# chao1224/pytorch_distributed_nn

Hardware: AMD Instinct MI355X
Metric: samples/sec (whole node) ResNet-50 DDP (higher is better)
Workload: dtype bf16; 1 GPU; model=resnet50 (ImageNet layout, 224x224, 1000 classes), global_batch=256, per_gpu_batch=256, image_size=224, parallelism=dp1, optimizer=fused SGD momentum=0.9 wd=5e-5, hipgraph=False, opt_overlap=False

## Files before the change

### csrc/kernels/conv3x3.hip

```cpp
#include "conv_direct.h"

namespace {
using namespace pg;

typedef __attribute__((ext_vector_type(8))) int c3v8i;
typedef __attribute__((ext_vector_type(4))) int c3v4i;
constexpr int C3_AMAX_PARTS = 1024;
#ifndef C3_PRE_J
#define C3_PRE_J 3
#endif
#ifndef C3_F8_PRE_J
#define C3_F8_PRE_J 2
#endif

template <int FMT>
__device__ __forceinline__ uint4 c3_to_fp8(const float* v) {
    constexpr float MX = FMT ? 57344.f : 448.f;
    int w[4];
#pragma unroll
    for (int d = 0; d < 4; ++d) {
        const float c0 = fminf(fmaxf(v[4 * d], -MX), MX), c1 = fminf(fmaxf(v[4 * d + 1], -MX), MX);
        const float c2 = fminf(fmaxf(v[4 * d + 2], -MX), MX), c3 = fminf(fmaxf(v[4 * d + 3], -MX), MX);
        int x = 0;
        if constexpr (FMT) {
            x = __builtin_amdgcn_cvt_pk_bf8_f32(c0, c1, x, false);
            x = __builtin_amdgcn_cvt_pk_bf8_f32(c2, c3, x, true);
        } else {
            x = __builtin_amdgcn_cvt_pk_fp8_f32(c0, c1, x, false);
            x = __builtin_amdgcn_cvt_pk_fp8_f32(c2, c3, x, true);
        }
        w[d] = x;
    }
    return make_uint4((uint32_t)w[0], (uint32_t)w[1], (uint32_t)w[2], (uint32_t)w[3]);
}

template <int NB, int EPI, bool PRE, int F8 = 0, bool FP = false>
__global__ void __launch_bounds__(256, 2) conv3x3_kernel(C3Args a) {
    constexpr int FN = NB / 16;
    constexpr int BCH = NB * 8 / 256;
    extern __shared__ __attribute__((aligned(16))) char smem[];
    bf16_t* const halo = reinterpret_cast<bf16_t*>(smem);
    bf16_t* const bbuf = halo + (a.halo_max + 1) * 64;

    const int tid = threadIdx.x, lane = tid & 63, wave = tid >> 6;
    const int t = xcd_remap(blockIdx.x, a.tiles * a.ntiles);
    const int tile = t / a.ntiles, nt = t - tile * a.ntiles;
    const int p0 = tile * C3_BM, n0 = nt * NB;
    const int plast = min(a.P, p0 + C3_BM) - 1;
    const int gr0 = (int)fdiv((uint32_t)p0, a.dW), gr1 = (int)fdiv((uint32_t)plast, a.dW);
    const int nrows = gr1 - gr0 + 3;
    const int hpx = nrows * a.W;
    const long gp0 = (long)(gr0 - 1) * a.W;

    int hb[4], py[4], px[4];
    bool pv[4];
#pragma unroll
    for (int f = 0; f < 4; ++f) {
        const int p = p0 + wave * 64 + f * 16 + (lane & 15);
        pv[f] = p < a.P;
        const int pp = pv[f] ? p : plast;
        const int gr = (int)fdiv((uint32_t)pp, a.dW);
        px[f] = pp - gr * a.W;
        py[f] = gr - (int)fdiv((uint32_t)gr, a.dH) * a.H;
        hb[f] = (gr - gr0 + 1) * a.W + px[f];
    }

    [[maybe_unused]] uint32_t tmask[4];
    if constexpr (F8 != 0) {
#pragma unroll
        for (int f = 0; f < 4; ++f) {
            uint32_t m = 0;
#pragma unroll
            for (int tap = 0; tap < 9; ++tap) {
                const int dr = tap / 3 - 1, ds = tap % 3 - 1;
                if (pv[f] && (unsigned)(py[f] + dr) < (unsigned)a.H && (unsigned)(px[f] + ds) < (unsigned)a.W) m |= 1u << tap;
            }
            tmask[f] = m;
        }
    }
    const int zpx = a.halo_max;
    if (tid < 8) *reinterpret_cast<u16x8_t*>(halo + zpx * 64 + tid * 8) = c3_zero8();

    f32x4_t acc[4][FN];
#pragma unroll
    for (int i = 0; i < 4; ++i)
#pragma unroll
        for (int j = 0; j < FN; ++j) acc[i][j] = f32x4_t{0.f, 0.f, 0.f, 0.f};

    const int nchunks = F8 ? a.C >> 7 : a.C >> 6;
    const long wrow = 9L * a.C;
    u16x8_t rb[BCH];
    [[maybe_unused]] const uint8_t* wb8 =
        reinterpret_cast<const uint8_t*>(a.w) + (long)(n0 + (tid >> 3)) * wrow + (tid & 7) * 16;
    auto load_b = [&](int c0, int tap) {
#pragma unroll
        for (int i = 0; i < BCH; ++i) {
            const int li = tid + 256 * i, row = li >> 3, q = li & 7;
            if constexpr (F8 != 0)
                rb[i] = *reinterpret_cast<const u16x8_t*>(wb8 + (long)(32 * i) * wrow + (long)tap * a.C + c0);
            else
                rb[i] = *reinterpret_cast<const u16x8_t*>(a.w + (long)(n0 + row) * wrow + (long)tap * a.C + c0 + q * 8);
        }
    };
    auto store_b = [&](int buf) {
        bf16_t* B = bbuf + buf * NB * 64;
#pragma unroll
        for (int i = 0; i < BCH; ++i) {
            const int li = tid + 256 * i, row = li >> 3, q = li & 7;
            *reinterpret_cast<u16x8_t*>(B + kimg_off(row, q)) = rb[i];
        }
    };

    [[maybe_unused]] float qs = 0.f, amx = 0.f;
    if constexpr (F8 != 0) qs = a.f8_scale[0];

    for (int ck = 0; ck < nchunks; ++ck) {
        const int c0 = F8 ? ck << 7 : ck << 6;
        if (ck) __syncthreads();
        const int nch = hpx * 8;
        if constexpr (F8 != 0) {
            constexpr int J = PRE ? C3_F8_PRE_J : 4;
            [[maybe_unused]] float* coef = reinterpret_cast<float*>(bbuf + NB * 64);
            if constexpr (PRE) {
                pre_coef_lds<128>(a, c0, coef, tid);
                __syncthreads();
            } else if constexpr (FP) {
                fpro_coef_lds<128>(a, c0, coef, tid);
                __syncthreads();
            }
            for (int i0 = 0; i0 < nch; i0 += 256 * J) {
                u16x8_t v[J][2], tv[PRE ? J : 1][2];
                bool okj[J];
                int gpj[J];
#pragma unroll
                for (int j = 0; j < J; ++j) {
                    const int i = i0 + j * 256 + tid;
                    const long gp = gp0 + (i >> 3);
                    okj[j] = i < nch && gp >= 0 && gp < a.P;
                    const long gc = gp < 0 ? 0 : (gp >= a.P ? a.P - 1 : gp);
                    gpj[j] = (int)gc;
                    const bf16_t* src = a.x + gc * a.C + c0 + (i & 7) * 16;
                    v[j][0] = *reinterpret_cast<const u16x8_t*>(src);
                    v[j][1] = *reinterpret_cast<const u16x8_t*>(src + 8);
                    if constexpr (PRE) {
                        const bf16_t* ts = a.pre_t + gc * a.C + c0 + (i & 7) * 16;
                        tv[j][0] = *reinterpret_cast<const u16x8_t*>(ts);
                        tv[j][1] = *reinterpret_cast<const u16x8_t*>(ts + 8);
                    }
                }
#pragma unroll
                for (int j = 0; j < J; ++j) {
                    if constexpr (PRE) {
#pragma unroll
                        for (int h = 0; h < 2; ++h) {
                            v[j][h] = pre_apply_lds<128>(coef, (tid & 7) * 16 + 8 * h, v[j][h], tv[j][h]);
                            if (a.pre_out && nt == 0 && okj[j] && gpj[j] >= p0 && gpj[j] <= plast)
                                *reinterpret_cast<u16x8_t*>(a.pre_out + (long)gpj[j] * a.C + c0 + (tid & 7) * 16 + 8 * h) =
                                    v[j][h];
                        }
                    }
                    if constexpr (FP) {
                        v[j][0] = fpro_apply_lds<128>(coef, (tid & 7) * 16, v[j][0]);
                        v[j][1] = fpro_apply_lds<128>(coef, (tid & 7) * 16 + 8, v[j][1]);
                    }
                    float f[16];
                    unpack8(v[j][0], f);
                    unpack8(v[j][1], f + 8);
                    float m = 0.f;
#pragma unroll
                    for (int e = 0; e < 16; ++e) {
                        m = fmaxf(m, fabsf(f[e]));
                        f[e] *= qs;
                    }
                    if (okj[j]) amx = fmaxf(amx, m);
                    const uint4 q8 = c3_to_fp8<F8 - 1>(f);
                    const int i = i0 + j * 256 + tid;
                    const int off = i < nch ? halo_off(i >> 3, i & 7) : zpx * 64 + (i & 7) * 8;
                    *reinterpret_cast<u16x8_t*>(halo + off) = mask16(__builtin_bit_cast(u16x8_t, q8), okj[j]);
                }
            }
            load_b(c0, 0);
            store_b(0);
            __syncthreads();
            const int g = lane >> 4;
#pragma unroll 1
            for (int tap = 0; tap < 9; ++tap) {
                const int dr = tap / 3 - 1, ds = tap - (tap / 3) * 3 - 1;
                load_b(c0, tap < 8 ? tap + 1 : 8);
                const bf16_t* B = bbuf + (tap & 1) * NB * 64;
                c3v8i bq[FN];
#pragma unroll
                for (int f = 0; f < FN; ++f) {
                    const int row = f * 16 + (lane & 15);
                    const c3v4i lo = *reinterpret_cast<const c3v4i*>(B + kimg_off(row, 2 * g));
                    const c3v4i hi = *reinterpret_cast<const c3v4i*>(B + kimg_off(row, 2 * g + 1));
                    bq[f] = c3v8i{lo[0], lo[1], lo[2], lo[3], hi[0], hi[1], hi[2], hi[3]};
                }
#pragma unroll
                for (int fm = 0; fm < 4; ++fm) {
                    const bool v = (tmask[fm] >> tap) & 1;
                    const int hp = v ? hb[fm] + dr * a.W + ds : zpx;
                    const c3v4i lo = *reinterpret_cast<const c3v4i*>(halo + halo_off(hp, 2 * g));
                    const c3v4i hi = *reinterpret_cast<const c3v4i*>(halo + halo_off(hp, 2 * g + 1));
                    const c3v8i af = c3v8i{lo[0], lo[1], lo[2], lo[3], hi[0], hi[1], hi[2], hi[3]};
#pragma unroll
                    for (int fn = 0; fn < FN; ++fn)
                        acc[fm][fn] = __builtin_amdgcn_mfma_scale_f32_16x16x128_f8f6f4(
                            bq[fn], af, acc[fm][fn], 0, F8 - 1, 0, 0x7f7f7f7f, 0, 0x7f7f7f7f);
                }
                store_b((tap + 1) & 1);
                __syncthreads();
            }
            continue;
        }
        constexpr int J = PRE ? (NB == 128 ? C3_PRE_J : 4) : 8;
        [[maybe_unused]] float* coef = reinterpret_cast<float*>(bbuf + NB * 64);
        if constexpr (PRE) {
            pre_coef_lds<64>(a, c0, coef, tid);
            __syncthreads();
        } else if constexpr (FP) {
            fpro_coef_lds<64>(a, c0, coef, tid);
            __syncthreads();
        }
        for (int i0 = 0; i0 < nch; i0 += 256 * J) {
            u16x8_t v[J], tv[PRE ? J : 1];
            bool okj[J];
            int gpj[J];
#pragma unroll
            for (int j = 0; j < J; ++j) {
                const int i = i0 + j * 256 + tid;
                const long gp = gp0 + (i >> 3);
                okj[j] = i < nch && gp >= 0 && gp < a.P;
                const long gc = gp < 0 ? 0 : (gp >= a.P ? a.P - 1 : gp);
                gpj[j] = (int)gc;
                v[j] = *reinterpret_cast<const u16x8_t*>(a.x + gc * a.C + c0 + (i & 7) * 8);
                if constexpr (PRE) tv[j] = *reinterpret_cast<const u16x8_t*>(a.pre_t + gc * a.C + c0 + (i & 7) * 8);
            }
#pragma unroll
            for (int j = 0; j < J; ++j) {
                if constexpr (PRE) {
                    v[j] = pre_apply_lds<64>(coef, (tid & 7) * 8, v[j], tv[j]);
                    if (a.pre_out && nt == 0 && okj[j] && gpj[j] >= p0 && gpj[j] <= plast)
                        *reinterpret_cast<u16x8_t*>(a.pre_out + (long)gpj[j] * a.C + c0 + (tid & 7) * 8) = v[j];
                }
                if constexpr (FP) v[j] = fpro_apply_lds<64>(coef, (tid & 7) * 8, v[j]);
                v[j] = mask16(v[j], okj[j]);
            }
#pragma unroll
            for (int j = 0; j < J; ++j) {
                const int i = i0 + j * 256 + tid;
                const int off = i < nch ? halo_off(i >> 3, i & 7) : zpx * 64 + (i & 7) * 8;
                *reinterpret_cast<u16x8_t*>(halo + off) = v[j];
            }
        }
        load_b(c0, 0);
        store_b(0);
        __syncthreads();
#pragma unroll 1
        for (int tap = 0; tap < 9; ++tap) {
            const int dr = tap / 3 - 1, ds = tap - (tap / 3) * 3 - 1;
            if (tap < 8) load_b(c0, tap + 1);
            int hp[4];
#pragma unroll
            for (int f = 0; f < 4; ++f) {
                const bool v = pv[f] && (unsigned)(py[f] + dr) < (unsigned)a.H && (unsigned)(px[f] + ds) < (unsigned)a.W;
                hp[f] = v ? hb[f] + dr * a.W + ds : zpx;
            }
            const bf16_t* B = bbuf + (tap & 1) * NB * 64;
#pragma unroll 1
            for (int ks = 0; ks < 2; ++ks) {
                bf16x8_t af[4], bfr[FN];
                const int q = ks * 4 + (lane >> 4);
#pragma unroll
                for (int f = 0; f < 4; ++f)
                    af[f] = __builtin_bit_cast(bf16x8_t, *reinterpret_cast<const u16x8_t*>(halo + halo_off(hp[f], q)));
#pragma unroll
                for (int f = 0; f < FN; ++f) bfr[f] = frag_kmajor(B, f * 16 + (lane & 15), ks, lane);
#pragma unroll
                for (int fm = 0; fm < 4; ++fm)
#pragma unroll
                    for (int fn = 0; fn < FN; ++fn)
                        acc[fm][fn] = __builtin_amdgcn_mfma_f32_16x16x32_bf16(bfr[fn], af[fm], acc[fm][fn], 0, 0, 0);
            }
            if (tap < 8) {
                store_b((tap + 1) & 1);
                __syncthreads();
            }
        }
    }

    if constexpr (F8 != 0) {
        amx = wave_max(amx);
        if (lane == 0)
            atomicMax(reinterpret_cast<unsigned int*>(a.f8_amax + (blockIdx.x & (C3_AMAX_PARTS - 1))), __float_as_uint(amx));
        const float gs = a.f8_inv[0] * a.f8_winv[0];
#pragma unroll
        for (int i = 0; i < 4; ++i)
#pragma unroll
            for (int j = 0; j < FN; ++j)
#pragma unroll
                for (int e = 0; e < 4; ++e) acc[i][j][e] *= gs;
    }
    c3_epilogue<NB, EPI>(a, acc, tile, p0, n0, wave, lane, pv);
}

constexpr int C3R_HREG = 16;

template <int EPI>
__global__ void __launch_bounds__(256, 1) conv3x3_w64_kernel(C3Args a) {
    constexpr int NB = 64, FN = 4;
    extern __shared__ __attribute__((aligned(16))) char smem[];
    bf16_t* const halo = reinterpret_cast<bf16_t*>(smem);
    bf16_t* const wres = halo + (a.halo_max + 1) * 64;
    const int tid = threadIdx.x, lane = tid & 63, wave = tid >> 6;
    const int zpx = a.halo_max;

    for (int i = tid; i < 9 * 64 * 8; i += 256) {
        const int tap = i / 512, row = (i >> 3) & 63, q = i & 7;
        *reinterpret_cast<u16x8_t*>(wres + tap * 4096 + kimg_off(row, q)) =
            *reinterpret_cast<const u16x8_t*>(a.w + (long)row * 576 + tap * 64 + q * 8);
    }
    if (tid < 8) *reinterpret_cast<u16x8_t*>(halo + zpx * 64 + tid * 8) = c3_zero8();

    u16x8_t hreg[C3R_HREG];
    auto tile_geom = [&](int tile, int& gr0, int& nch, long& gp0) {
        const int p0 = tile * C3_BM;
        const int plast = min(a.P, p0 + C3_BM) - 1;
        gr0 = (int)fdiv((uint32_t)p0, a.dW);
        const int gr1 = (int)fdiv((uint32_t)plast, a.dW);
        nch = (gr1 - gr0 + 3) * a.W * 8;
        gp0 = (long)(gr0 - 1) * a.W;
    };
    auto fetch = [&](int tile) {
        int gr0, nch;
        long gp0;
        tile_geom(tile, gr0, nch, gp0);
#pragma unroll
        for (int j = 0; j < C3R_HREG; ++j) {
            const int i = j * 256 + tid;
            const long gp = gp0 + (i >> 3);
            const bool ok = i < nch && gp >= 0 && gp < a.P;
            const long gc = gp < 0 ? 0 : (gp >= a.P ? a.P - 1 : gp);
            const u16x8_t ld = *reinterpret_cast<const u16x8_t*>(a.x + gc * 64 + (i & 7) * 8);
            hreg[j] = mask16(ld, ok);
        }
    };
    auto put = [&](int tile) {
        int gr0, nch;
        long gp0;
        tile_geom(tile, gr0, nch, gp0);
#pragma unroll
        for (int j = 0; j < C3R_HREG; ++j) {
            const int i = j * 256 + tid;
            const int off = i < nch ? halo_off(i >> 3, i & 7) : zpx * 64 + (i & 7) * 8;
            *reinterpret_cast<u16x8_t*>(halo + off) = hreg[j];
        }
    };

    int tile = blockIdx.x;
    if (tile < a.tiles) fetch(tile);
    for (; tile < a.tiles; tile += gridDim.x) {
        __syncthreads();
        put(tile);
        __syncthreads();
        const int next = tile + gridDim.x;
        if (next < a.tiles) fetch(next);

        int gr0, nch;
        long gp0;
        tile_geom(tile, gr0, nch, gp0);
        const int p0 = tile * C3_BM;
        const int plast = min(a.P, p0 + C3_BM) - 1;
        int hb[4], py[4], px[4];
        bool pv[4];
#pragma unroll
        for (int f = 0; f < 4; ++f) {
            const int p = p0 + wave * 64 + f * 16 + (lane & 15);
            pv[f] = p < a.P;
            const int pp = pv[f] ? p : plast;
            const int gr = (int)fdiv((uint32_t)pp, a.dW);
            px[f] = pp - gr * a.W;
            py[f] = gr - (int)fdiv((uint32_t)gr, a.dH) * a.H;
            hb[f] = (gr - gr0 + 1) * a.W + px[f];
        }
        f32x4_t acc[4][FN];
#pragma unroll
        for (int i = 0; i < 4; ++i)
#pragma unroll
            for (int j = 0; j < FN; ++j) acc[i][j] = f32x4_t{0.f, 0.f, 0.f, 0.f};
#pragma unroll
        for (int tap = 0; tap < 9; ++tap) {
            const int dr = tap / 3 - 1, ds = tap % 3 - 1;
            int hp[4];
#pragma unroll
            for (int f = 0; f < 4; ++f) {
                const bool v = pv[f] && (unsigned)(py[f] + dr) < (unsigned)a.H && (unsigned)(px[f] + ds) < (unsigned)a.W;
                hp[f] = v ? hb[f] + dr * a.W + ds : zpx;
            }
            const bf16_t* B = wres + tap * 4096;
#pragma unroll
            for (int ks = 0; ks < 2; ++ks) {
                bf16x8_t af[4], bfr[FN];
                const int q = ks * 4 + (lane >> 4);
#pragma unroll
                for (int f = 0; f < 4; ++f)
                    af[f] = __builtin_bit_cast(bf16x8_t, *reinterpret_cast<const u16x8_t*>(halo + halo_off(hp[f], q)));
#pragma unroll
                for (int f = 0; f < FN; ++f) bfr[f] = frag_kmajor(B, f * 16 + (lane & 15), ks, lane);
#pragma unroll
                for (int fm = 0; fm < 4; ++fm)
#pragma unroll
                    for (int fn = 0; fn < FN; ++fn)
                        acc[fm][fn] = __builtin_amdgcn_mfma_f32_16x16x32_bf16(bfr[fn], af[fm], acc[fm][fn], 0, 0, 0);
            }
        }
        c3_epilogue<NB, EPI>(a, acc, tile, p0, 0, wave, lane, pv);
    }
}

template <int KC, int NB, int EPI, bool PRE, bool FP = false>
__global__ void __launch_bounds__(256, 2) conv1x1_areg_kernel(C3Args a) {
    constexpr int FN = NB / 16, NKS = 2 * KC, K = 64 * KC;
    constexpr int BPT = NB * KC * 8 / 256;
    static_assert(BPT >= 1 && NB * KC * 8 % 256 == 0, "weight step must cover the block");
    extern __shared__ __attribute__((aligned(16))) char smem[];
    bf16_t* const bbuf = reinterpret_cast<bf16_t*>(smem);
    const int tid = threadIdx.x, lane = tid & 63, wave = tid >> 6;
    const int groups = a.ntiles;
    const int t = xcd_remap(blockIdx.x, a.tiles * groups);
    const int tile = t / groups, grp = t - tile * groups;
    const int steps = (a.N / NB) / groups;
    const int c00 = grp * steps;
    const int p0 = tile * C3_BM;

    u16x8_t rb[BPT];
    auto load_b = [&](int s) {
        const int n0 = (c00 + s) * NB;
#pragma unroll
        for (int i = 0; i < BPT; ++i) {
            const int li = tid + 256 * i, row = li / (KC * 8), rem = li - row * (KC * 8);
            rb[i] = *reinterpret_cast<const u16x8_t*>(a.w + (long)(n0 + row) * K + rem * 8);
        }
    };
    auto store_b = [&](int buf) {
        bf16_t* B = bbuf + buf * (KC * NB * 64);
#pragma unroll
        for (int i = 0; i < BPT; ++i) {
            const int li = tid + 256 * i, row = li / (KC * 8), rem = li - row * (KC * 8);
            *reinterpret_cast<u16x8_t*>(B + (rem >> 3) * (NB * 64) + kimg_off(row, rem & 7)) = rb[i];
        }
    };
    load_b(0);

    bool pv[4];
    long prow[4];
#pragma unroll
    for (int fm = 0; fm < 4; ++fm) {
        const int p = p0 + wave * 64 + fm * 16 + (lane & 15);
        pv[fm] = p < a.P;
        prow[fm] = (long)(pv[fm] ? p : a.P - 1) * K;
    }
    bf16x8_t af[NKS][4];
    if constexpr (!PRE) {
        [[maybe_unused]] float* coef = reinterpret_cast<float*>(bbuf + 2 * KC * NB * 64);
        if constexpr (FP) {
            for (int c = tid; c < K; c += 256) {
                coef[c] = a.pro_sc[c];
                coef[K + c] = a.pro_sh[c];
            }
            __syncthreads();
        }
#pragma unroll
        for (int ks = 0; ks < NKS; ++ks)
#pragma unroll
            for (int fm = 0; fm < 4; ++fm) {
                u16x8_t v = *reinterpret_cast<const u16x8_t*>(a.x + prow[fm] + ks * 32 + (lane >> 4) * 8);
                if constexpr (FP) v = fpro_apply_lds<K>(coef, ks * 32 + (lane >> 4) * 8, v);
                af[ks][fm] = __builtin_bit_cast(bf16x8_t, v);
            }
    } else {
        float* coef = reinterpret_cast<float*>(bbuf + 2 * KC * NB * 64);
        {
            const float invL = (float)(1.0 / (double)a.P);
            for (int c = tid; c < K; c += 256) {
                const float is = a.pre_invstd[c], kk = (a.pre_gamma ? a.pre_gamma[c] : 1.f) * is;
                const float dg = a.pre_dgamma[c] * invL, db = a.pre_dbeta[c] * invL;
                coef[c] = kk;
                coef[K + c] = -kk * is * dg;
                coef[2 * K + c] = kk * (a.pre_mean[c] * is * dg - db);
            }
        }
        __syncthreads();
        constexpr int GB = KC == 4 ? 2 : (KC == 2 ? 4 : 2);
#pragma unroll
        for (int g0 = 0; g0 < NKS; g0 += GB) {
            u16x8_t v[GB][4], tv[GB][4];
#pragma unroll
            for (int kk = 0; kk < GB; ++kk)
#pragma unroll
                for (int fm = 0; fm < 4; ++fm) {
                    const long off = prow[fm] + (g0 + kk) * 32 + (lane >> 4) * 8;
                    v[kk][fm] = *reinterpret_cast<const u16x8_t*>(a.x + off);
                    tv[kk][fm] = *reinterpret_cast<const u16x8_t*>(a.pre_t + off);
                }
#pragma unroll
            for (int kk = 0; kk < GB; ++kk) {
                const int k = (g0 + kk) * 32 + (lane >> 4) * 8;
                PreCoef pc;
#pragma unroll
                for (int j = 0; j < 8; ++j) {
                    pc.k[j] = coef[k + j];
                    pc.A[j] = coef[K + k + j];
                    pc.B[j] = coef[2 * K + k + j];
                }
#pragma unroll
                for (int fm = 0; fm < 4; ++fm) {
                    const u16x8_t d = pre_apply(pc, v[kk][fm], tv[kk][fm]);
                    if (a.pre_out && grp == 0 && pv[fm]) *reinterpret_cast<u16x8_t*>(a.pre_out + prow[fm] + k) = d;
                    af[g0 + kk][fm] = __builtin_bit_cast(bf16x8_t, d);
                }
            }
        }
    }
    store_b(0);
    __syncthreads();

    for (int s = 0; s < steps; ++s) {
        const bool more = s + 1 < steps;
        if (more) load_b(s + 1);
        const bf16_t* B = bbuf + (s & 1) * (KC * NB * 64);
        f32x4_t acc[4][FN];
#pragma unroll
        for (int i = 0; i < 4; ++i)
#pragma unroll
            for (int j = 0; j < FN; ++j) acc[i][j] = f32x4_t{0.f, 0.f, 0.f, 0.f};
        bf16x8_t bcur[FN], bnxt[FN];
#pragma unroll
        for (int f = 0; f < FN; ++f) bcur[f] = frag_kmajor(B, f * 16 + (lane & 15), 0, lane);
#pragma unroll
        for (int ks = 0; ks < NKS; ++ks) {
            if (ks + 1 < NKS) {
#pragma unroll
                for (int f = 0; f < FN; ++f)
                    bnxt[f] = frag_kmajor(B + ((ks + 1) >> 1) * (NB * 64), f * 16 + (lane & 15), (ks + 1) & 1, lane);
            }
#pragma unroll
            for (int fm = 0; fm < 4; ++fm)
#pragma unroll
                for (int fn = 0; fn < FN; ++fn)
                    acc[fm][fn] = __builtin_amdgcn_mfma_f32_16x16x32_bf16(bcur[fn], af[ks][fm], acc[fm][fn], 0, 0, 0);
            __builtin_amdgcn_sched_barrier(0);
#pragma unroll
            for (int f = 0; f < FN; ++f) bcur[f] = bnxt[f];
        }
        if (more) store_b((s + 1) & 1);
        c3_epilogue<NB, EPI>(a, acc, tile, p0, (c00 + s) * NB, wave, lane, pv);
        if (more) __syncthreads();
    }
}

int c3r_smem(int W);

__global__ void __launch_bounds__(256) conv3x3_flip_kernel(const bf16_t* __restrict__ w, bf16_t* __restrict__ wt,
                                                           int K, int C) {
    const long n = 9L * K * C;
    for (long i = (long)blockIdx.x * 256 + threadIdx.x; i < n; i += (long)gridDim.x * 256) {
        const int c = (int)(i % C);
        const long r1 = i / C;
        const int tap = (int)(r1 % 9);
        const int k = (int)(r1 / 9);
        wt[((long)c * 9 + (8 - tap)) * K + k] = w[i];
    }
}

int c3_halo_max(int W) {
    const int rows = (C3_BM - 1 + W - 1) / W + 1 + 2;
    return rows * W;
}

__global__ void __launch_bounds__(256) conv3x3_flip8_kernel(const uint8_t* __restrict__ w, uint8_t* __restrict__ wt,
                                                            int K, int C) {
    const long n = 9L * K * C;
    for (long i = (long)blockIdx.x * 256 + threadIdx.x; i < n; i += (long)gridDim.x * 256) {
        const int k = (int)(i % K);
        const long r0 = i / K;
        const int tap = (int)(r0 % 9), c = (int)(r0 / 9);
        wt[i] = w[((long)k * 9 + (8 - tap)) * C + c];
    }
}

template <int NB>
int c3_smem(int W) { return (c3_halo_max(W) + 1) * 128 + 2 * NB * 128; }

int c3r_smem(int W) { return (c3_halo_max(W) + 1) * 128 + 9 * 64 * 128; }

template <int EPI>
int c3r_launch(const C3Args& a, hipStream_t st) {
    static int attr_done = 0;
    const int sm = c3r_smem(a.W);
    if (sm > attr_done) {
        (void)hipFuncSetAttribute((const void*)conv3x3_w64_kernel<EPI>, hipFuncAttributeMaxDynamicSharedMemorySize, sm);
        attr_done = sm;
    }
    const int grid = a.tiles < grid_cus() ? a.tiles : grid_cus();
    hipLaunchKernelGGL((conv3x3_w64_kernel<EPI>), dim3(grid), dim3(256), sm, st, a);
    PDNN_LAUNCH_RET;
}

template <int NB, int EPI, bool PRE, int F8 = 0, bool FP = false>
int c3_launch(const C3Args& a, hipStream_t st) {
    static int attr_done = 0;
    const int sm = c3_smem<NB>(a.W);
    if (sm > attr_done) {
        (void)hipFuncSetAttribute((const void*)conv3x3_kernel<NB, EPI, PRE, F8, FP>,
                                  hipFuncAttributeMaxDynamicSharedMemorySize, sm);
        attr_done = sm;
    }
    hipLaunchKernelGGL((conv3x3_kernel<NB, EPI, PRE, F8, FP>), dim3(a.tiles * a.ntiles), dim3(256), sm, st, a);
    PDNN_LAUNCH_RET;
}

template <int NB, bool PRE>
int c3_dispatch(const C3Args& a, int epi, hipStream_t st) {
    switch (epi) {
        case C3_BNB: return c3_launch<NB, C3_BNB, PRE>(a, st);
        case C3_STATS: return c3_launch<NB, C3_STATS, PRE>(a, st);
        case C3_RES: return c3_launch<NB, C3_RES, PRE>(a, st);
        default: return c3_launch<NB, C3_PLAIN, PRE>(a, st);
    }
}

}



template <int KC, int NB, int EPI, bool PRE, bool FP = false>
int areg_launch(const C3Args& a, hipStream_t st) {
    constexpr int sm = 2 * KC * NB * 128 + (PRE ? 3 * 64 * KC * 4 : (FP ? 2 * 64 * KC * 4 : 0));
    hipLaunchKernelGGL((conv1x1_areg_kernel<KC, NB, EPI, PRE, FP>), dim3(a.tiles * a.ntiles), dim3(256), sm, st, a);
    PDNN_LAUNCH_RET;
}

template <int KC, int NB, bool PRE>
int areg_dispatch(const C3Args& a, int epi, hipStream_t st) {
    if constexpr (!PRE) {
        if (a.pro_sc) {
            if (epi == C3_STATS) return areg_launch<KC, NB, C3_STATS, false, true>(a, st);
            if (epi == C3_PLAIN) return areg_launch<KC, NB, C3_PLAIN, false, true>(a, st);
            return (int)hipErrorInvalidValue;
        }
    }
    switch (epi) {
        case C3_BNB: return areg_launch<KC, NB, C3_BNB, PRE>(a, st);
        case C3_STATS: return areg_launch<KC, NB, C3_STATS, PRE>(a, st);
        case C3_RES: return areg_launch<KC, NB, C3_RES, PRE>(a, st);
        default: return areg_launch<KC, NB, C3_PLAIN, PRE>(a, st);
    }
}

template <bool PRE>
int areg_run(C3Args& a, int K, int epi, hipStream_t st) {
    const int nb = K == 256 ? 32 : 64;
    const int chunks = a.N / nb;
    int g = 1;
    while (g < chunks && (long)a.tiles * g < 512 && chunks % (2 * g) == 0) g *= 2;
    a.ntiles = g;
    if (K == 64) return areg_dispatch<1, 64, PRE>(a, epi, st);
    if (K == 128) return areg_dispatch<2, 64, PRE>(a, epi, st);
    return areg_dispatch<4, 32, PRE>(a, epi, st);
}

static bool set_pre(C3Args& a, const bf16_t* t, const float* mean, const float* invstd, const float* gamma,
             const float* dgamma, const float* dbeta, bf16_t* out) {
    a.pre_t = t; a.pre_mean = mean; a.pre_invstd = invstd; a.pre_gamma = gamma;
    a.pre_dgamma = dgamma; a.pre_dbeta = dbeta; a.pre_out = out;
    if (!t) return !out;
    return mean && invstd && dgamma && dbeta;
}
static int c3_force() { return pg::tune().conv3x3_force; }

static FastDiv make_fdiv_c3(uint32_t d) {
    FastDiv f;
    f.d = d ? d : 1;
    uint32_t l = 0;
    while ((1ull << l) < f.d) ++l;
    f.s = l;
    f.m = (uint32_t)((((1ull << l) - f.d) << 32) / f.d + 1);
    return f;
}

PDNN_API int pdnn_conv3x3_supported(int Nimg, int H, int W, int C, int N) {
    if (C % 64 || N % 64 || C < 64 || N < 64 || W < 1 || H < 1) return 0;
    if (W < 12 && !c3_force()) return 0;
    if ((long)Nimg * H * W >= (1L << 31) / 2) return 0;
    const int nb = N % 128 == 0 ? 128 : 64;
    const int sm = nb == 128 ? c3_smem<128>(W) : c3_smem<64>(W);
    return sm <= 80 * 1024 ? 1 : 0;
}

PDNN_API int pdnn_conv3x3_force(int f) {
    const int old = c3_force();
    pg::tune().conv3x3_force = f ? 1 : 0;
    return old;
}

PDNN_API int pdnn_conv3x3_stats_rows(int Nimg, int H, int W) {
    return (int)cdiv((long)Nimg * H * W, C3_BM) * 4;
}

PDNN_API int pdnn_conv3x3_flip_tiled(const bf16_t* w, bf16_t* wt, int K, int C, hipStream_t st);

PDNN_API int pdnn_conv3x3_flip(const bf16_t* w, bf16_t* wt, int K, int C, hipStream_t st) {
    if (K % 8 == 0 && C % 8 == 0) return pdnn_conv3x3_flip_tiled(w, wt, K, C, st);
    hipLaunchKernelGGL(conv3x3_flip_kernel, dim3(stream_grid(9L * K * C, 256)), dim3(256), 0, st, w, wt, K, C);
    PDNN_LAUNCH_RET;
}

PDNN_API int pdnn_conv3x3_flip8(const uint8_t* w, uint8_t* wt, int K, int C, hipStream_t st) {
    hipLaunchKernelGGL(conv3x3_flip8_kernel, dim3(stream_grid(9L * K * C, 256)), dim3(256), 0, st, w, wt, K, C);
    PDNN_LAUNCH_RET;
}

PDNN_API int pdnn_conv3x3(const bf16_t* x, const bf16_t* w, bf16_t* y, int Nimg, int H, int W, int C, int N,
                          float* stats, const bf16_t* res, const uint8_t* res_mask, const bf16_t* bn_x,
                          const float* bn_mean,
                          const float* bn_invstd, const float* bn_mscale, const float* bn_mshift, int nb,
                          const bf16_t* pre_t, const float* pre_mean, const float* pre_invstd,
                          const float* pre_gamma, const float* pre_dgamma, const float* pre_dbeta, bf16_t* pre_out,
                          const float* pro_sc, const float* pro_sh, hipStream_t st) {
    if (!pdnn_conv3x3_supported(Nimg, H, W, C, N)) return (int)hipErrorInvalidValue;
    C3Args a{};
    a.x = x; a.w = w; a.y = y;
    a.Nimg = Nimg; a.H = H; a.W = W; a.C = C; a.N = N; a.P = Nimg * H * W;
    a.dW = make_fdiv_c3(W); a.dH = make_fdiv_c3(H);
    a.tiles = (int)cdiv(a.P, C3_BM);
    a.halo_max = c3_halo_max(W);
    a.stats = stats; a.res = res; a.rmask = res_mask;
    if (res_mask && !res) return (int)hipErrorInvalidValue;
    if (!set_pre(a, pre_t, pre_mean, pre_invstd, pre_gamma, pre_dgamma, pre_dbeta, pre_out))
        return (int)hipErrorInvalidValue;
    const bool pre = pre_t != nullptr;
    a.ep_x = bn_x; a.ep_mean = bn_mean; a.ep_invstd = bn_invstd; a.ep_mscale = bn_mscale; a.ep_mshift = bn_mshift;
    const int epi = bn_x ? C3_BNB : (stats ? C3_STATS : (res ? C3_RES : C3_PLAIN));
    if (bn_x && !stats) return (int)hipErrorInvalidValue;
    if (!pro_sc != !pro_sh) return (int)hipErrorInvalidValue;
    if (pro_sc) {
        if (pre || (epi != C3_STATS && epi != C3_PLAIN)) return (int)hipErrorInvalidValue;
        a.pro_sc = pro_sc; a.pro_sh = pro_sh;
        if (nb <= 1) nb = N % 128 == 0 ? 128 : 64;
        if (nb == 128 && (N % 128 || c3_smem<128>(W) > 80 * 1024)) nb = 64;
        a.ntiles = N / nb;
        if (nb == 128)
            return epi == C3_STATS ? c3_launch<128, C3_STATS, false, 0, true>(a, st) : c3_launch<128, C3_PLAIN, false, 0, true>(a, st);
        return epi == C3_STATS ? c3_launch<64, C3_STATS, false, 0, true>(a, st) : c3_launch<64, C3_PLAIN, false, 0, true>(a, st);
    }
    if (nb == 1 && !pre && C == 64 && N == 64 && c3_halo_max(W) * 8 <= C3R_HREG * 256 &&
        c3r_smem(W) <= 160 * 1024) {
        a.ntiles = 1;
        switch (epi) {
            case C3_BNB: return c3r_launch<C3_BNB>(a, st);
            case C3_STATS: return c3r_launch<C3_STATS>(a, st);
            case C3_RES: return c3r_launch<C3_RES>(a, st);
            default: return c3r_launch<C3_PLAIN>(a, st);
        }
    }
    if (nb == 0 || nb == 1) nb = N % 128 == 0 ? 128 : 64;
    if (nb == 128 && (N % 128 || c3_smem<128>(W) > 80 * 1024)) nb = 64;
    a.ntiles = N / nb;
    if (nb == 128) return pre ? c3_dispatch<128, true>(a, epi, st) : c3_dispatch<128, false>(a, epi, st);
    return pre ? c3_dispatch<64, true>(a, epi, st) : c3_dispatch<64, false>(a, epi, st);
}

PDNN_API int pdnn_conv3x3_fp8_supported(int Nimg, int H, int W, int C, int N) {
    return pdnn_conv3x3_supported(Nimg, H, W, C, N) && C % 128 == 0 && N % 128 == 0 &&
           c3_smem<128>(W) <= 80 * 1024;
}

PDNN_API int pdnn_conv3x3_fp8(const bf16_t* x, const uint8_t* wq, bf16_t* y, int Nimg, int H, int W, int C, int N,
                              float* stats, const bf16_t* bn_x, const float* bn_mean, const float* bn_invstd,
                              const float* bn_mscale, const float* bn_mshift, const bf16_t* pre_t,
                              const float* pre_mean, const float* pre_invstd, const float* pre_gamma,
                              const float* pre_dgamma, const float* pre_dbeta, bf16_t* pre_out, const float* scale,
                              const float* inv, const float* winv, float* amax, int e5m2, const float* pro_sc,
                              const float* pro_sh, hipStream_t st) {
    if (!pdnn_conv3x3_fp8_supported(Nimg, H, W, C, N) || !scale || !inv || !winv || !amax)
        return (int)hipErrorInvalidValue;
    C3Args a{};
    a.x = x; a.w = reinterpret_cast<const bf16_t*>(wq); a.y = y;
    a.Nimg = Nimg; a.H = H; a.W = W; a.C = C; a.N = N; a.P = Nimg * H * W;
    a.dW = make_fdiv_c3(W); a.dH = make_fdiv_c3(H);
    a.tiles = (int)cdiv(a.P, C3_BM);
    a.halo_max = c3_halo_max(W);
    a.stats = stats;
    if (!set_pre(a, pre_t, pre_mean, pre_invstd, pre_gamma, pre_dgamma, pre_dbeta, pre_out))
        return (int)hipErrorInvalidValue;
    a.ep_x = bn_x; a.ep_mean = bn_mean; a.ep_invstd = bn_invstd; a.ep_mscale = bn_mscale; a.ep_mshift = bn_mshift;
    if (bn_x && !stats) return (int)hipErrorInvalidValue;
    a.f8_scale = scale; a.f8_inv = inv; a.f8_winv = winv; a.f8_amax = amax;
    a.ntiles = N / 128;
    const bool pre = pre_t != nullptr;
    if (e5m2) {
        if (bn_x) return pre ? c3_launch<128, C3_BNB, true, 2>(a, st) : c3_launch<128, C3_BNB, false, 2>(a, st);
        if (stats) return (int)hipErrorInvalidValue;
        return pre ? c3_launch<128, C3_PLAIN, true, 2>(a, st) : c3_launch<128, C3_PLAIN, false, 2>(a, st);
    }
    if (pre || bn_x) return (int)hipErrorInvalidValue;
    if (!pro_sc != !pro_sh) return (int)hipErrorInvalidValue;
    if (pro_sc) {
        a.pro_sc = pro_sc; a.pro_sh = pro_sh;
        return stats ? c3_launch<128, C3_STATS, false, 1, true>(a, st) : c3_launch<128, C3_PLAIN, false, 1, true>(a, st);
    }
    return stats ? c3_launch<128, C3_STATS, false, 1>(a, st) : c3_launch<128, C3_PLAIN, false, 1>(a, st);
}

PDNN_API int pdnn_conv1x1_panel_supported(long P, int K, int N) {
    const bool k_ok = K == 64 || K == 128 || K == 256;
    return k_ok && N % 64 == 0 && N >= 64 && P > 0 && P < (1L << 30) ? 1 : 0;
}

PDNN_API int pdnn_conv1x1_panel(const bf16_t* x, const bf16_t* w, bf16_t* y, long P, int K, int N, float* stats,
                                const bf16_t* res, const uint8_t* res_mask, const bf16_t* bn_x, const float* bn_mean,
                                const float* bn_invstd, const float* bn_mscale, const float* bn_mshift,
                                const bf16_t* pre_t, const float* pre_mean, const float* pre_invstd,
                                const float* pre_gamma, const float* pre_dgamma, const float* pre_dbeta,
                                bf16_t* pre_out, const float* pro_sc, const float* pro_sh, hipStream_t st) {
    if (!pdnn_conv1x1_panel_supported(P, K, N) || (bn_x && !stats) || (res_mask && !res) || (!pro_sc != !pro_sh) ||
        (pro_sc && (pre_t || bn_x || res)))
        return (int)hipErrorInvalidValue;
    C3Args a{};
    a.x = x; a.w = w; a.y = y; a.C = K; a.N = N; a.P = (int)P;
    a.tiles = (int)cdiv(P, C3_BM);
    a.stats = stats; a.res = res; a.rmask = res_mask;
    a.ep_x = bn_x; a.ep_mean = bn_mean; a.ep_invstd = bn_invstd; a.ep_mscale = bn_mscale; a.ep_mshift = bn_mshift;
    if (!set_pre(a, pre_t, pre_mean, pre_invstd, pre_gamma, pre_dgamma, pre_dbeta, pre_out))
        return (int)hipErrorInvalidValue;
    a.pro_sc = pro_sc; a.pro_sh = pro_sh;
    const int epi = bn_x ? C3_BNB : (stats ? C3_STATS : (res ? C3_RES : C3_PLAIN));
    return pre_t ? areg_run<true>(a, K, epi, st) : areg_run<false>(a, K, epi, st);
}

PDNN_API int pdnn_conv1x1_panel_stats_rows(long P) { return (int)cdiv(P, C3_BM) * 4; }
```

Baseline: 12190 samples/s.

## Raise 1x1 areg conv occupancy for KC=1 plain and cost-model the group split

Measured after the change: 12220 samples/s, median of 6. About the same (+0.3%).

```diff
diff --git a/csrc/kernels/conv3x3.hip b/csrc/kernels/conv3x3.hip
--- a/csrc/kernels/conv3x3.hip
+++ b/csrc/kernels/conv3x3.hip
@@ -418,10 +418,13 @@
     }
 }
 
+constexpr int areg_bpc(int KC, int EPI) { return KC == 1 && EPI == C3_PLAIN ? 3 : 2; }
+
 template <int KC, int NB, int EPI, bool PRE, bool FP = false>
-__global__ void __launch_bounds__(256, 2) conv1x1_areg_kernel(C3Args a) {
+__global__ void __launch_bounds__(256, areg_bpc(KC, EPI)) conv1x1_areg_kernel(C3Args a) {
     constexpr int FN = NB / 16, NKS = 2 * KC, K = 64 * KC;
     constexpr int BPT = NB * KC * 8 / 256;
+    constexpr bool BPF = areg_bpc(KC, EPI) == 2;
     static_assert(BPT >= 1 && NB * KC * 8 % 256 == 0, "weight step must cover the block");
     extern __shared__ __attribute__((aligned(16))) char smem[];
     bf16_t* const bbuf = reinterpret_cast<bf16_t*>(smem);
@@ -438,8 +441,9 @@
         const int n0 = (c00 + s) * NB;
 #pragma unroll
         for (int i = 0; i < BPT; ++i) {
-            const int li = tid + 256 * i, row = li / (KC * 8), rem = li - row * (KC * 8);
-            rb[i] = *reinterpret_cast<const u16x8_t*>(a.w + (long)(n0 + row) * K + rem * 8);
+            constexpr int RPP = 256 / (KC * 8);
+            const bf16_t* wu = a.w + (long)(n0 + i * RPP) * K;
+            rb[i] = *reinterpret_cast<const u16x8_t*>(wu + (unsigned)tid * 8u);
         }
     };
     auto store_b = [&](int buf) {
@@ -533,13 +537,21 @@
 #pragma unroll
         for (int i = 0; i < 4; ++i)
 #pragma unroll
-            for (int j = 0; j < FN; ++j) acc[i][j] = f32x4_t{0.f, 0.f, 0.f, 0.f};
+            for (int j = 0; j < FN; ++j) {
+                acc[i][j] = f32x4_t{0.f, 0.f, 0.f, 0.f};
+            }
         bf16x8_t bcur[FN], bnxt[FN];
 #pragma unroll
         for (int f = 0; f < FN; ++f) bcur[f] = frag_kmajor(B, f * 16 + (lane & 15), 0, lane);
 #pragma unroll
         for (int ks = 0; ks < NKS; ++ks) {
-            if (ks + 1 < NKS) {
+            if constexpr (!BPF) {
+                if (ks > 0) {
+#pragma unroll
+                    for (int f = 0; f < FN; ++f)
+                        bcur[f] = frag_kmajor(B + (ks >> 1) * (NB * 64), f * 16 + (lane & 15), ks & 1, lane);
+                }
+            } else if (ks + 1 < NKS) {
 #pragma unroll
                 for (int f = 0; f < FN; ++f)
                     bnxt[f] = frag_kmajor(B + ((ks + 1) >> 1) * (NB * 64), f * 16 + (lane & 15), (ks + 1) & 1, lane);
@@ -550,8 +562,10 @@
                 for (int fn = 0; fn < FN; ++fn)
                     acc[fm][fn] = __builtin_amdgcn_mfma_f32_16x16x32_bf16(bcur[fn], af[ks][fm], acc[fm][fn], 0, 0, 0);
             __builtin_amdgcn_sched_barrier(0);
-#pragma unroll
-            for (int f = 0; f < FN; ++f) bcur[f] = bnxt[f];
+            if constexpr (BPF) {
+#pragma unroll
+                for (int f = 0; f < FN; ++f) bcur[f] = bnxt[f];
+            }
         }
         if (more) store_b((s + 1) & 1);
         c3_epilogue<NB, EPI>(a, acc, tile, p0, (c00 + s) * NB, wave, lane, pv);
@@ -637,6 +651,7 @@
 template <int KC, int NB, int EPI, bool PRE, bool FP = false>
 int areg_launch(const C3Args& a, hipStream_t st) {
     constexpr int sm = 2 * KC * NB * 128 + (PRE ? 3 * 64 * KC * 4 : (FP ? 2 * 64 * KC * 4 : 0));
+    static_assert(sm * areg_bpc(KC, EPI) <= 160 * 1024, "the resident blocks' LDS must fit the CU");
     hipLaunchKernelGGL((conv1x1_areg_kernel<KC, NB, EPI, PRE, FP>), dim3(a.tiles * a.ntiles), dim3(256), sm, st, a);
     PDNN_LAUNCH_RET;
 }
@@ -659,12 +674,24 @@
 }
 
 template <bool PRE>
+int areg_groups(int tiles, int chunks, int K, int nb, int epi) {
+    const int kc = K / 64;
+    const long slots = (long)grid_cus() * areg_bpc(kc, epi);
+    const long load = (PRE ? 2 : 1) * K, step = (epi == C3_RES || epi == C3_BNB ? 2 : 1) * nb;
+    int best = 1;
+    long best_cost = 0;
+    for (int g = 1; g <= chunks && chunks % g == 0; g *= 2) {
+        const long rounds = ((long)tiles * g + slots - 1) / slots;
+        const long cost = rounds * (load + (chunks / g) * step);
+        if (g == 1 || cost < best_cost) { best = g; best_cost = cost; }
+    }
+    return best;
+}
+
+template <bool PRE>
 int areg_run(C3Args& a, int K, int epi, hipStream_t st) {
     const int nb = K == 256 ? 32 : 64;
-    const int chunks = a.N / nb;
-    int g = 1;
-    while (g < chunks && (long)a.tiles * g < 512 && chunks % (2 * g) == 0) g *= 2;
-    a.ntiles = g;
+    a.ntiles = areg_groups<PRE>(a.tiles, a.N / nb, K, nb, epi);
     if (K == 64) return areg_dispatch<1, 64, PRE>(a, epi, st);
     if (K == 128) return areg_dispatch<2, 64, PRE>(a, epi, st);
     return areg_dispatch<4, 32, PRE>(a, epi, st);
```
